# intel/edge-video-analytics-microservice

Measured on AMD Instinct MI355X. Metric: pre-processed frames/sec (1080p NV12→512² NCHW fp32) 1–8 GPU; % HBM peak, higher is better.
Workload: dtype u8->f32; 1 GPU; C2: 32x 1920x1080 NV12 (pitch 1920, device-resident) -> 32x3x512x512 fp32 NCHW, range [0,1] + mean/std; items_per_launch=32, src=1920x1080 NV12, dst=512x512, pool_sets=5, pool_bytes=1000980480, launches_in_flight=3, parallelism=streams s mod 1, one process per GPU, no hot-loop collective

## Files before the change

### edge-video-analytics-microservice_amd/csrc/evam_pp.hip

```cpp
#include <hip/hip_runtime.h>

#include <algorithm>
#include <cmath>
#include <cstdarg>
#include <cstddef>
#include <cstdint>
#include <cstdio>
#include <cstring>
#include <map>
#include <tuple>
#include <mutex>
#include <string>
#include <type_traits>
#include <vector>
#include <immintrin.h>

#include "../../include/evam_pp.h"

#define EVAM_HD __host__ __device__
#include "evam_geom.h"
#include "evam_rings.h"
#include "evam_clip_simd.h"
#include "evam_jpeg_dec.h"
#include "evam_track.h"
// ... 1323 lines not shown
        }
        asm volatile("" ::: "memory");
        int v[3][PX];
        if (cur.pad || (kAblate & 2)) {
#pragma unroll
            for (int j = 0; j < PX; j++) { v[0][j] = fb0; v[1][j] = fo1; v[2][j] = fb2; }
        } else {
            uint32_t NA[PX][3], NB[PX][3];
            const bool shareC = kYUV && cur.stA && cur.stB && !cur.stCB;
            if (shareC) {
                if constexpr (kYUV) hrow2(buf, buf + oY1, buf + oC0, buf + oV0, NA, NB);
            } else {
                if (cur.stA) hrow(buf, buf + oC0, buf + oV0, NA);
                else {
#pragma unroll
                    for (int j = 0; j < PX; j++)
#pragma unroll
                        for (int ch = 0; ch < 3; ch++) NA[j][ch] = cur.ya == pa ? HA[j][ch] : HB[j][ch];
                }
                if (cur.stB) hrow(buf + oY1, buf + (cur.stCB ? oC1 : oC0), buf + (cur.stCB ? oV1 : oV0), NB);
                else {
#pragma unroll
                    for (int j = 0; j < PX; j++)
#pragma unroll
                        for (int ch = 0; ch < 3; ch++)
                            NB[j][ch] = cur.yb == cur.ya ? NA[j][ch] : (cur.yb == pa ? HA[j][ch] : HB[j][ch]);
                }
            }
            const uint32_t wb0 = (uint32_t)cur.b0, wb1 = (uint32_t)cur.b1;
#pragma unroll
            for (int j = 0; j < PX; j++) {
                const bool padc = wa[j] == 0;
#pragma unroll
                for (int ch = 0; ch < 3; ch++) {
                    const int r = vresize(NA[j][ch], NB[j][ch], wb0, wb1);
                    v[ch][j] = padc ? (ch == 0 ? fb0 : (ch == 1 ? fo1 : fb2)) : r;
                }
            }
            if (REUSE) {
#pragma unroll
                for (int j = 0; j < PX; j++)
#pragma unroll
                    for (int ch = 0; ch < 3; ch++) { HA[j][ch] = NA[j][ch]; HB[j][ch] = NB[j][ch]; }
            }
        }
        store_row(Y, v);
        asm volatile("" ::: "memory");
        pa = na;
        pb = nb;
        cur = nxt;
    }
}

#ifdef EVAM_PP_TRACE
constexpr int kTraceWGs = 16384, kTraceSlots = 12;
__device__ unsigned long long g_evam_trace[kTraceWGs * kTraceSlots];
#define EVAM_STAMP(k)                                                                                  \
    do {                                                                                               \
        unsigned long long t_;                                                                         \
        __builtin_amdgcn_sched_barrier(0);                                                             \
        asm volatile("s_memrealtime %0\n\ts_waitcnt lgkmcnt(0)" : "=s"(t_)::"memory");               \
        __builtin_amdgcn_sched_barrier(0);                                                             \
        if (threadIdx.x == 0 && blockIdx.x < kTraceWGs) g_evam_trace[blockIdx.x * kTraceSlots + (k)] = t_; \
    } while (0)
#define EVAM_TRACE_VAL(k, v)                                                                           \
    do {                                                                                               \
        if (threadIdx.x == 0 && blockIdx.x < kTraceWGs) g_evam_trace[blockIdx.x * kTraceSlots + (k)] = (v); \
    } while (0)
#define EVAM_WSTAMP(k)                                                                                 \
    do {                                                                                               \
        unsigned long long t_;                                                                         \
        __builtin_amdgcn_sched_barrier(0);                                                             \
        asm volatile("s_memrealtime %0\n\ts_waitcnt lgkmcnt(0)" : "=s"(t_)::"memory");               \
        __builtin_amdgcn_sched_barrier(0);                                                             \
        const unsigned w_ = ((blockIdx.z * gridDim.y + blockIdx.y) * gridDim.x + blockIdx.x) * (blockDim.x >> 6) + (threadIdx.x >> 6); \
        if ((threadIdx.x & 63) == 0 && w_ < (unsigned)kTraceWGs) g_evam_trace[w_ * kTraceSlots + (k)] = t_; \
    } while (0)
#define EVAM_WTRACE_VAL(k, v)                                                                          \
    do {                                                                                               \
        const unsigned w_ = ((blockIdx.z * gridDim.y + blockIdx.y) * gridDim.x + blockIdx.x) * (blockDim.x >> 6) + (threadIdx.x >> 6); \
        if ((threadIdx.x & 63) == 0 && w_ < (unsigned)kTraceWGs) g_evam_trace[w_ * kTraceSlots + (k)] = (v); \
    } while (0)
#else
#define EVAM_STAMP(k) do { } while (0)
#define EVAM_TRACE_VAL(k, v) do { } while (0)
#define EVAM_WSTAMP(k) do { } while (0)
#define EVAM_WTRACE_VAL(k, v) do { } while (0)
#endif

static_assert(sizeof(evam_roi) == 20, "evam_roi layout");

struct alignas(64) RoiRec {
    const uint8_t* plane[3];
    int32_t pitch[3];
    uint16_t width, height;
    int32_t x, y, w, h;
    int32_t item;
    uint16_t row0, row1;
};
static_assert(sizeof(RoiRec) == 64, "RoiRec layout");
static_assert(offsetof(RoiRec, x) == 40 && offsetof(RoiRec, item) == 56 && offsetof(RoiRec, row0) == 60, "RoiRec lines");
static_assert(offsetof(evam_roi, h) == offsetof(evam_roi, x) + 12, "evam_roi rect");
struct RecFrame { __m128i l[3]; };

constexpr int kMaxStrips = 32;
constexpr int kSfoot = 64;
constexpr int strip_slot(int fmt, int px) { return px == 1 && fmt != kBGRX ? 512 : 1024; }

struct TParams {
    ItemArg items[kArgItems];
    double scale_x, scale_y;
    const float* lut;
    void* dst;
    int slot_offset, slot_stride;
    int DW, DH;
    int cw, ch, rw, rh, ox, oy;
    int nw;
    int TH, tiles_x, tiles_per_item;
    int wave_bytes;
    int color_rgb;
    uint32_t fill;
    int2 sfoot[kSfoot];
    int nstrips, units;
    int segY, segC;
    int nrY;
    int prio;
    int ahead;
};
static_assert(sizeof(TParams) <= 4000, "strip / band kernel arguments must fit the 4 KB kernarg segment");

struct ProgressPrio {
    int next, q2, q3, level;
    __device__ __forceinline__ ProgressPrio(bool on, int n) : next(on ? n / 4 : -1), q2(n / 2), q3((3 * n) / 4), level(3) {
        if (on) __builtin_amdgcn_s_setprio(3);
    }
    __device__ __forceinline__ void step(int i) {
        if (__builtin_expect(i != next, 1)) return;
        if (level == 3) {
            __builtin_amdgcn_s_setprio(2);
            level = 2;
            next = q2;
        } else if (level == 2) {
            __builtin_amdgcn_s_setprio(1);
            level = 1;
            next = q3;
        } else {
            __builtin_amdgcn_s_setprio(0);
            level = 0;
            next = -1;
        }
    }
};

template <int FMT, int OUT, int D, int PX, int PR, bool NHWC = false>
__global__ __launch_bounds__(512) void evam_pp_strip(const TParams P) {
    static_assert(!NHWC || OUT == 1, "the interleaved strip store is fp32 only");
    constexpr int NS = NHWC ? 1 : 3;
    __shared__ __attribute__((aligned(16))) float lut_s[OUT != 0 ? 768 : 4];
    extern __shared__ __attribute__((aligned(16))) uint8_t smem[];
    static_assert(FMT == kNV12 || FMT == kI420 || FMT == kBGRX, "4:2:0 or BGRx sources");
    static_assert(D >= 1 && D <= 4, "ring depth");
    static_assert(PX == 1 || PX == 2, "pixels per lane");
    constexpr int SLOT = strip_slot(FMT, PX);
    constexpr bool PK = FMT == kBGRX;
    constexpr int NPC = FMT == kI420 ? 2 : (PK ? 0 : 1);
    static_assert(PR == 0 || PR == 1, "paired taps");
    constexpr int NMIN = PR ? (PK ? 1 : 2) : 2 + NPC;
    const int lane = threadIdx.x & 63;
    const int wave = __builtin_amdgcn_readfirstlane(threadIdx.x >> 6);
    if (kAblate & 128) return;
    EVAM_WSTAMP(0);
    const uint8_t *p0, *p1, *p2;
    int pitch0, pitch1, pitch2, x0, y0, index, p_nw, p_DH, p_DW, strip, Y0, Y1;
    int g_ox, g_rw, g_oy, g_rh, g_cw, k_ch, k_rgb;
    double k_scale_x, k_scale_y;
    const float* k_lut;
    int2 sf;
    const int item = blockIdx.z, ty = blockIdx.y;
    const ItemArg& it = P.items[item];
    sf = P.sfoot[min((int)blockIdx.x * 8 + wave, kSfoot - 1)];
    const int p_TH = P.TH;
    p_nw = P.nw; p_DH = P.DH; p_DW = P.DW;
    p0 = it.plane[0];
    p1 = it.plane[1];
    p2 = it.plane[2];
    pitch0 = it.pitch[0]; pitch1 = it.pitch[1]; pitch2 = it.pitch[2];
    x0 = it.x0; y0 = it.y0;
    index = it.index;
    asm volatile("" ::"s"(p_nw), "s"(p_TH), "s"(p_DH), "s"(p_DW), "s"(P.ox), "s"(P.rw), "s"(P.oy), "s"(P.rh),
                 "s"(P.wave_bytes), "s"(p0), "s"(p1), "s"(p2), "s"(pitch0), "s"(pitch1), "s"(pitch2), "s"(x0), "s"(y0),
                 "s"(index), "s"(sf.x), "s"(sf.y), "s"(P.dst), "s"(P.slot_offset), "s"(P.slot_stride));
    k_scale_y = P.scale_y;
    k_ch = P.ch; k_rgb = P.color_rgb;
    k_lut = P.lut;
    asm volatile("" : "+s"(k_scale_y), "+s"(k_ch), "+s"(k_lut), "+s"(k_rgb));
    strip = (int)blockIdx.x * p_nw + wave;
    Y0 = ty * p_TH; Y1 = min(Y0 + p_TH, p_DH);
    g_ox = P.ox; g_rw = P.rw; g_oy = P.oy; g_rh = P.rh; g_cw = P.cw;
    k_scale_x = P.scale_x;
    const int X0 = strip * 64 * PX;
    const bool live = X0 < p_DW;
    const bool cols = live && sf.x >= 0;
    int fsY = 0, nY = 0, fsC = 0, nC = 0;
    if (cols) footprint_chunks(FMT, PK ? 4 : 1, x0 + sf.x, x0 + sf.y, fsY, nY, fsC, nC);
    const int vr0 = max(Y0, g_oy), vr1 = min(Y1, g_oy + g_rh);
    const int n = cols && vr1 > vr0 ? vr1 - vr0 : 0;

    int lr0 = 0, lr1 = 0, lb0 = 0, lb1 = 0;
    if (lane < n) {
        int sy, b0, b1;
        linear_coef(vr0 + lane - g_oy, k_scale_y, k_ch, false, sy, b0, b1);
        lr0 = min(max(sy, 0), k_ch - 1);
        lr1 = min(max(sy + 1, 0), k_ch - 1);
        lb0 = b0 << 8;
        lb1 = b1 << 8;
    }
    const __amdgpu_buffer_rsrc_t rsY = __builtin_amdgcn_make_buffer_rsrc((void*)p0, (short)0, 0x7FFFFFFF, 0x00020000);
    const __amdgpu_buffer_rsrc_t rsU = __builtin_amdgcn_make_buffer_rsrc((void*)p1, (short)0, 0x7FFFFFFF, 0x00020000);
    const __amdgpu_buffer_rsrc_t rsV = __builtin_amdgcn_make_buffer_rsrc((void*)(NPC == 2 ? p2 : p1), (short)0, 0x7FFFFFFF, 0x00020000);
    uint8_t* const wbuf = smem + wave * P.wave_bytes;
    constexpr int SY = PR ? 512 : SLOT;
    constexpr int CB = PR ? 1024 : 2 * SLOT;
    constexpr int SC = PR ? (NPC == 2 ? 256 : 512) : SLOT;
    constexpr int SV = PR ? 512 : 2 * SLOT;
    constexpr int GRP = PR ? (PK ? 1024 : 2048) : 2 * SLOT + 2 * NPC * SLOT;
    constexpr int segY = SY;
    const uint8_t* const pcl = NPC == 2 && PR ? (p1 < p2 ? p1 : p2) : p1;
    const uint32_t dU = (uint32_t)(p1 - pcl), dV = (uint32_t)(p2 - pcl);
    const __amdgpu_buffer_rsrc_t rsC2 = __builtin_amdgcn_make_buffer_rsrc((void*)pcl, (short)0, 0x7FFFFFFF, 0x00020000);
    auto issue = [&](int i, int k) {
        if (kAblate & 16) return;
        const int ya = y0 + __builtin_amdgcn_readlane(lr0, i), yb = y0 + __builtin_amdgcn_readlane(lr1, i);
        uint8_t* e = wbuf + k * GRP;
        if constexpr (PR) {
            const int hi = lane >> 5, c = lane & 31;
            if (c < nY)
                __builtin_amdgcn_raw_ptr_buffer_load_lds(rsY, (__attribute__((address_space(3))) void*)e, 16,
                                                         (uint32_t)((hi ? yb : ya) * pitch0 + fsY + c * 16), 0,
                                                         EVAM_PP_LOAD_AUX, 0);
            if constexpr (NPC == 1) {
                const int ca = ya >> 1, cb = yb >> 1;
                if (c < nC && (!hi || ca != cb))
                    __builtin_amdgcn_raw_ptr_buffer_load_lds(rsU, (__attribute__((address_space(3))) void*)(e + CB), 16,
                                                             (uint32_t)((hi ? cb : ca) * pitch1 + fsC + c * 16), 0,
                                                             EVAM_PP_LOAD_AUX, 0);
            } else if constexpr (NPC == 2) {
                const int ca = ya >> 1, cb = yb >> 1, q = lane >> 4, c4 = lane & 15, r = (q & 1) ? cb : ca;
                const uint32_t off = (q & 2) ? dV + (uint32_t)(r * pitch2) : dU + (uint32_t)(r * pitch1);
                if (c4 < nC && (!(q & 1) || ca != cb))
                    __builtin_amdgcn_raw_ptr_buffer_load_lds(rsC2, (__attribute__((address_space(3))) void*)(e + CB), 16,
                                                             off + (uint32_t)(fsC + c4 * 16), 0, EVAM_PP_LOAD_AUX, 0);
            }
            return;
        }
        const uint32_t vo = (uint32_t)lane * 16u;
        if (lane < nY) {
            __builtin_amdgcn_raw_ptr_buffer_load_lds(rsY, (__attribute__((address_space(3))) void*)e, 16, vo,
                                                     ya * pitch0 + fsY, EVAM_PP_LOAD_AUX, 0);
            __builtin_amdgcn_raw_ptr_buffer_load_lds(rsY, (__attribute__((address_space(3))) void*)(e + segY), 16, vo,
                                                     yb * pitch0 + fsY, EVAM_PP_LOAD_AUX, 0);
        }
        if constexpr (NPC == 0) return;
        const int ca = ya >> 1, cb = yb >> 1;
        if (lane < nC) {
            __builtin_amdgcn_raw_ptr_buffer_load_lds(rsU, (__attribute__((address_space(3))) void*)(e + CB), 16, vo,
                                                     ca * pitch1 + fsC, EVAM_PP_LOAD_AUX, 0);
            if constexpr (NPC == 2)
                __builtin_amdgcn_raw_ptr_buffer_load_lds(rsV, (__attribute__((address_space(3))) void*)(e + CB + SV),
                                                         16, vo, ca * pitch2 + fsC, EVAM_PP_LOAD_AUX, 0);
        }
        if (ca != cb && lane < nC) {
            __builtin_amdgcn_raw_ptr_buffer_load_lds(rsU, (__attribute__((address_space(3))) void*)(e + CB + SC), 16,
                                                     vo, cb * pitch1 + fsC, EVAM_PP_LOAD_AUX, 0);
            if constexpr (NPC == 2)
                __builtin_amdgcn_raw_ptr_buffer_load_lds(rsV, (__attribute__((address_space(3))) void*)(e + CB + SV + SC),
                                                         16, vo, cb * pitch2 + fsC, EVAM_PP_LOAD_AUX, 0);
        }
    };

    const int nthr = p_nw * 64;
    const bool lut_early = nthr >= 256;
    if constexpr (OUT != 0) {
        if (lut_early && wave < 3) {
            const __amdgpu_buffer_rsrc_t rsL = __builtin_amdgcn_make_buffer_rsrc((void*)k_lut, (short)0, 3072, 0x00020000);
            __builtin_amdgcn_raw_ptr_buffer_load_lds(rsL, (__attribute__((address_space(3))) void*)(lut_s + wave * 256), 16,
                                                     (uint32_t)lane * 16u, (k_rgb ? 2 - wave : wave) * 1024, 0, 0);
        }
    }
    const int npro = min(n, D);
    for (int i = 0; i < npro; i++) issue(i, i);
    EVAM_WSTAMP(1);
    EVAM_WTRACE_VAL(5, (unsigned long long)blockIdx.z | ((unsigned long long)strip << 16) |
                           ((unsigned long long)blockIdx.y << 32) | ((unsigned long long)n << 48));

    bool xin[PX], padc[PX];
    uint32_t lY[PX], lC0[PX], lC1[PX], wp[PX], vo[PX];
    bool anyp = false;
    const size_t esz = out_esz(OUT);
#pragma unroll
    for (int j = 0; j < PX; j++) {
        const int X = X0 + lane + 64 * j;
        xin[j] = live && X < p_DW;
        vo[j] = (uint32_t)(xin[j] ? X : 0) * (uint32_t)(NHWC ? 3 * esz : esz);
        lY[j] = lC0[j] = lC1[j] = wp[j] = 0;
        padc[j] = true;
        const int dx = X - g_ox;
        if (cols && xin[j] && dx >= 0 && dx < g_rw) {
            int s0, a0, a1;
            linear_coef(dx, k_scale_x, g_cw, true, s0, a0, a1);
            const int ca = x0 + s0;
            lY[j] = (uint32_t)(ca * (PK ? 4 : 1) - fsY);
            if constexpr (FMT == kNV12) {
                lC0[j] = (uint32_t)(2 * (ca >> 1) - fsC);
                lC1[j] = (uint32_t)(2 * ((ca + 1) >> 1) - fsC);
            } else if constexpr (FMT == kI420) {
                lC0[j] = (uint32_t)((ca >> 1) - fsC);
                lC1[j] = (uint32_t)(((ca + 1) >> 1) - fsC);
            }
            wp[j] = PK ? ((uint32_t)a0 << 4) | ((uint32_t)a1 << 20) : (uint32_t)a0 | ((uint32_t)a1 << 16);
            padc[j] = false;
        }
        anyp |= xin[j] && padc[j];
    }
    const bool anypad = cols && __builtin_amdgcn_ballot_w64(anyp) != 0;
    const bool full = X0 + 64 * (PX - 1) < p_DW;

    const size_t plane = (size_t)p_DW * p_DH;
    uint8_t* const d0 = reinterpret_cast<uint8_t*>(P.dst) + (size_t)(P.slot_offset + index * P.slot_stride) * 3 * plane * esz;
    uint8_t* const d1 = d0 + plane * esz;
    uint8_t* const d2 = d1 + plane * esz;
    const __amdgpu_buffer_rsrc_t rsO0 = __builtin_amdgcn_make_buffer_rsrc((void*)(!NHWC && k_rgb ? d2 : d0), (short)0, 0x7FFFFFFF, 0x00020000);
    const __amdgpu_buffer_rsrc_t rsO1 = __builtin_amdgcn_make_buffer_rsrc((void*)d1, (short)0, 0x7FFFFFFF, 0x00020000);
    const __amdgpu_buffer_rsrc_t rsO2 = __builtin_amdgcn_make_buffer_rsrc((void*)(k_rgb ? d0 : d2), (short)0, 0x7FFFFFFF, 0x00020000);
    const uint32_t fq0 = P.fill & 0xFF, fq1 = (P.fill >> 8) & 0xFF, fq2 = (P.fill >> 16) & 0xFF;
    const uint32_t fsh = OUT != 0 ? 2 : 0;
    const uint32_t fill0 = (k_rgb ? fq2 : fq0) << fsh, fill1 = fq1 << fsh, fill2 = (k_rgb ? fq0 : fq2) << fsh;

    if constexpr (OUT != 0) {
        if (lut_early) {
            if (npro == D) asm volatile("s_waitcnt vmcnt(%0)" ::"n"(NMIN * D) : "memory");
            else vmcnt_exact(NMIN * npro);
            lds_barrier();
        } else {
            for (int idx = threadIdx.x; idx < 768; idx += nthr)
                lut_s[idx] = k_lut[k_rgb ? 512 - (idx & ~255) + (idx & 255) : idx];
            __syncthreads();
        }
    }
    EVAM_WSTAMP(2);
    if (!live) return;
    if (kAblate & 64) {
        asm volatile("s_waitcnt vmcnt(0)" ::: "memory");
        asm volatile("" ::"v"(lY[0]), "v"(lC0[0]), "v"(lC1[0]), "v"(wp[0]), "v"(vo[0]), "v"(lb0), "v"(lb1));
        return;
    }
    const uint8_t* lutb = reinterpret_cast<const uint8_t*>(lut_s);
    const uint8_t* aY[PX];
    const uint8_t* aC0[PX];
    const uint8_t* aC1[PX];
#pragma unroll
    for (int j = 0; j < PX; j++) {
        aY[j] = wbuf + lY[j];
        aC0[j] = wbuf + CB + lC0[j];
        aC1[j] = wbuf + CB + lC1[j];
    }
    uint32_t kb = kKBs, kg = kKGs, kr = kKRs;
    int cvg = kCVG, cug = kCUG;
    asm volatile("" : "+v"(kb), "+v"(kg), "+v"(kr), "+s"(cvg), "+s"(cug));
    auto uvt = [&](uint32_t U, uint32_t V) {
        int gu = __mul24((int)U, cug) + (int)kg;
        asm("" : "+v"(gu));
        return UVs{__umul24(U, (uint32_t)kCUB) + kb, (uint32_t)(__mul24((int)V, cvg) + gu), __umul24(V, (uint32_t)kCVR) + kr};
    };
    auto put = [&](int Y, int j, uint32_t v0, uint32_t v1, uint32_t v2) {
        if (!xin[j]) return;
        if (kAblate & 4) {
            asm volatile("" ::"v"(v0), "v"(v1), "v"(v2));
            return;
        }
        if constexpr (NHWC) {
            const int l0 = (int)*reinterpret_cast<const uint32_t*>(lutb + v0);
            const int l1 = (int)*reinterpret_cast<const uint32_t*>(lutb + 1024 + v1);
            const int l2 = (int)*reinterpret_cast<const uint32_t*>(lutb + 2048 + v2);
            const evam_v3i q = {k_rgb ? l2 : l0, l1, k_rgb ? l0 : l2};
            __builtin_amdgcn_raw_buffer_store_b96(q, rsO0, vo[j] + (uint32_t)(Y * p_DW) * 12u, 0, EVAM_PP_STORE_AUX);
            return;
        }
        const int so = (int)((uint32_t)(Y * p_DW) * (uint32_t)esz);
        if constexpr (OUT == 1) {
            __builtin_amdgcn_raw_buffer_store_b32(*reinterpret_cast<const uint32_t*>(lutb + v0), rsO0, vo[j], so, EVAM_PP_STORE_AUX);
            __builtin_amdgcn_raw_buffer_store_b32(*reinterpret_cast<const uint32_t*>(lutb + 1024 + v1), rsO1, vo[j], so, EVAM_PP_STORE_AUX);
            __builtin_amdgcn_raw_buffer_store_b32(*reinterpret_cast<const uint32_t*>(lutb + 2048 + v2), rsO2, vo[j], so, EVAM_PP_STORE_AUX);
        } else if constexpr (OUT == 2) {
            __builtin_amdgcn_raw_buffer_store_b16(*reinterpret_cast<const uint16_t*>(lutb + v0), rsO0, vo[j], so, EVAM_PP_STORE_AUX);
            __builtin_amdgcn_raw_buffer_store_b16(*reinterpret_cast<const uint16_t*>(lutb + 1024 + v1), rsO1, vo[j], so, EVAM_PP_STORE_AUX);
            __builtin_amdgcn_raw_buffer_store_b16(*reinterpret_cast<const uint16_t*>(lutb + 2048 + v2), rsO2, vo[j], so, EVAM_PP_STORE_AUX);
        } else {
            __builtin_amdgcn_raw_buffer_store_b8((uint8_t)v0, rsO0, vo[j], so, EVAM_PP_STORE_AUX);
            __builtin_amdgcn_raw_buffer_store_b8((uint8_t)v1, rsO1, vo[j], so, EVAM_PP_STORE_AUX);
            __builtin_amdgcn_raw_buffer_store_b8((uint8_t)v2, rsO2, vo[j], so, EVAM_PP_STORE_AUX);
        }
    };
    auto put_fill = [&](int Y) {
#pragma unroll
        for (int j = 0; j < PX; j++) put(Y, j, fill0, fill1, fill2);
    };
    const int ra = n ? vr0 : Y1;
    for (int Y = Y0; Y < ra; Y++) put_fill(Y);

    ProgressPrio prio(P.prio != 0, n);
    const int nst = full ? NS * PX : NS;
    auto row = [&](int i, int kk, auto has_pad) {
        constexpr bool PADC = decltype(has_pad)::value;
        constexpr int SD = D - 1;
        if (SD == 0) {
            asm volatile("s_waitcnt vmcnt(0)" ::: "memory");
        } else if (i >= SD && i + D - 1 < n) {
            if (PX == 1 || !full) asm volatile("s_waitcnt vmcnt(%0)" ::"n"((D - 1) * NMIN + SD * NS) : "memory");
            else asm volatile("s_waitcnt vmcnt(%0)" ::"n"((D - 1) * NMIN + SD * NS * PX) : "memory");
        } else {
            vmcnt_exact(NMIN * (min(i + D - 1, n - 1) - i) + nst * min(i, SD));
        }
#ifdef EVAM_PP_TRACE
        if (i == 0) EVAM_WSTAMP(3);
#endif
        prio.step(i);
        const int Y = vr0 + i;
        const uint32_t wb0 = (uint32_t)__builtin_amdgcn_readlane(lb0, i), wb1 = (uint32_t)__builtin_amdgcn_readlane(lb1, i);
        const int ya = __builtin_amdgcn_readlane(lr0, i), yb = __builtin_amdgcn_readlane(lr1, i);
        const bool share = ((y0 + ya) >> 1) == ((y0 + yb) >> 1);
        if (kAblate & 2) {
            put_fill(Y);
        } else if constexpr (PK) {
            const int eo = kk * GRP;
#pragma unroll
            for (int j = 0; j < PX; j++) {
                const uint32_t* ay = reinterpret_cast<const uint32_t*>(aY[j] + eo);
                const uint32_t qa0 = ay[0], qa1 = ay[1], qb0 = ay[SY / 4], qb1 = ay[SY / 4 + 1];
                uint32_t v[3];
#pragma unroll
                for (int c = 0; c < 3; c++) {
                    const uint32_t sel = 0x0C000C00u | ((uint32_t)(4 + c) << 16) | (uint32_t)c;
                    const uint32_t ha = __builtin_amdgcn_udot2(
                        __builtin_bit_cast(evam_u16x2, __builtin_amdgcn_perm(qa1, qa0, sel)),
                        __builtin_bit_cast(evam_u16x2, wp[j]), 0u, false);
                    const uint32_t hb = __builtin_amdgcn_udot2(
                        __builtin_bit_cast(evam_u16x2, __builtin_amdgcn_perm(qb1, qb0, sel)),
                        __builtin_bit_cast(evam_u16x2, wp[j]), 0u, false);
                    v[c] = vfinal<OUT>(ha, hb, wb0, wb1);
                }
                if constexpr (PADC) {
                    v[0] = padc[j] ? fill0 : v[0];
                    v[1] = padc[j] ? fill1 : v[1];
                    v[2] = padc[j] ? fill2 : v[2];
                }
                put(Y, j, v[0], v[1], v[2]);
            }
        } else {
            const int eo = kk * GRP;
            uint32_t rY[PX][4], rC[PX][2][2], rE[PX][2][2];
            auto raw_c = [&](const uint8_t* a, int o, uint32_t (&c)[2]) {
                c[0] = a[o];
                c[1] = FMT == kNV12 ? a[o + 1] : a[o + SV];
            };
#pragma unroll
            for (int j = 0; j < PX; j++) {
                const uint8_t* ay = aY[j] + eo;
                rY[j][0] = ay[0]; rY[j][1] = ay[1]; rY[j][2] = ay[SY]; rY[j][3] = ay[SY + 1];
                raw_c(aC0[j], eo, rC[j][0]);
                raw_c(aC1[j], eo, rC[j][1]);
            }
            if (!share) {
#pragma unroll
                for (int j = 0; j < PX; j++) {
                    raw_c(aC0[j], eo + SC, rE[j][0]);
                    raw_c(aC1[j], eo + SC, rE[j][1]);
                }
            }
#pragma unroll
            for (int j = 0; j < PX; j++) {
                const UVs tA = uvt(rC[j][0][0], rC[j][0][1]), tB = uvt(rC[j][1][0], rC[j][1][1]);
                const uint32_t yA = luma_term(rY[j][0]), yB = luma_term(rY[j][1]);
                const uint32_t yC = luma_term(rY[j][2]), yD = luma_term(rY[j][3]);
                uint32_t h0[3], h1[3];
                h0[0] = hpass_sat(yA, tA.b, yB, tB.b, wp[j]);
                h0[1] = hpass_sat(yA, tA.g, yB, tB.g, wp[j]);
                h0[2] = hpass_sat(yA, tA.r, yB, tB.r, wp[j]);
                if (share) {
                    h1[0] = hpass_sat(yC, tA.b, yD, tB.b, wp[j]);
                    h1[1] = hpass_sat(yC, tA.g, yD, tB.g, wp[j]);
                    h1[2] = hpass_sat(yC, tA.r, yD, tB.r, wp[j]);
                    asm volatile("; strip: shared chroma row" ::"v"(h1[0]), "v"(h1[1]), "v"(h1[2]));
                } else {
                    const UVs tC = uvt(rE[j][0][0], rE[j][0][1]), tE = uvt(rE[j][1][0], rE[j][1][1]);
                    h1[0] = hpass_sat(yC, tC.b, yD, tE.b, wp[j]);
                    h1[1] = hpass_sat(yC, tC.g, yD, tE.g, wp[j]);
                    h1[2] = hpass_sat(yC, tC.r, yD, tE.r, wp[j]);
                    asm volatile("; strip: two chroma rows" ::"v"(h1[0]), "v"(h1[1]), "v"(h1[2]));
                }
                uint32_t v[3];
#pragma unroll
                for (int c = 0; c < 3; c++) v[c] = vfinal<OUT>(h0[c], h1[c], wb0, wb1);
                if constexpr (PADC) {
                    v[0] = padc[j] ? fill0 : v[0];
                    v[1] = padc[j] ? fill1 : v[1];
                    v[2] = padc[j] ? fill2 : v[2];
                }
                put(Y, j, v[0], v[1], v[2]);
            }
        }
        asm volatile("" ::: "memory");
        if (i + D < n) issue(i + D, kk);
        asm volatile("" ::: "memory");
    };
    auto ring = [&](auto has_pad) {
        for (int i0 = 0; i0 < n; i0 += D) {
#pragma unroll
            for (int kk = 0; kk < D; kk++)
                if (i0 + kk < n) row(i0 + kk, kk, has_pad);
        }
    };
    if (anypad) ring(std::true_type{});
    else ring(std::false_type{});
    for (int Y = max(ra, vr1); Y < Y1; Y++) put_fill(Y);
#ifdef EVAM_PP_TRACE
    asm volatile("s_waitcnt vmcnt(0)" ::: "memory");
    EVAM_WSTAMP(4);
    {
        unsigned xcc;
        asm volatile("s_getreg_b32 %0, hwreg(HW_REG_XCC_ID)" : "=s"(xcc));
        EVAM_WTRACE_VAL(6, (unsigned long long)xcc);
    }
#endif
}

__device__ __forceinline__ void vmcnt_le(int n) {
    n = __builtin_amdgcn_readfirstlane(n);
    asm volatile(
        "s_cmp_lt_i32 %0, 8\n\t"
        "s_cbranch_scc1 5f\n\t"
        "s_cmp_lt_i32 %0, 16\n\t"
        "s_cbranch_scc1 2f\n\t"
        "s_cmp_lt_i32 %0, 32\n\t"
        "s_cbranch_scc1 1f\n\t"
        "s_waitcnt vmcnt(32)\n\t"
        "s_branch 9f\n"
        "1:\n\t"
        "s_waitcnt vmcnt(16)\n\t"
        "s_branch 9f\n"
        "2:\n\t"
        "s_cmp_lt_i32 %0, 12\n\t"
        "s_cbranch_scc1 3f\n\t"
        "s_waitcnt vmcnt(12)\n\t"
        "s_branch 9f\n"
        "3:\n\t"
        "s_waitcnt vmcnt(8)\n\t"
        "s_branch 9f\n"
        "5:\n\t"
        "s_cmp_lt_i32 %0, 4\n\t"
        "s_cbranch_scc1 7f\n\t"
        "s_cmp_lt_i32 %0, 6\n\t"
        "s_cbranch_scc1 6f\n\t"
        "s_waitcnt vmcnt(6)\n\t"
        "s_branch 9f\n"
        "6:\n\t"
        "s_waitcnt vmcnt(4)\n\t"
        "s_branch 9f\n"
        "7:\n\t"
        "s_cmp_lt_i32 %0, 2\n\t"
        "s_cbranch_scc1 8f\n\t"
        "s_cmp_lt_i32 %0, 3\n\t"
        "s_cbranch_scc1 4f\n\t"
        "s_waitcnt vmcnt(3)\n\t"
        "s_branch 9f\n"
        "4:\n\t"
        "s_waitcnt vmcnt(2)\n\t"
        "s_branch 9f\n"
        "8:\n\t"
        "s_cmp_lt_i32 %0, 1\n\t"
        "s_cbranch_scc1 10f\n\t"
        "s_waitcnt vmcnt(1)\n\t"
        "s_branch 9f\n"
        "10:\n\t"
        "s_waitcnt vmcnt(0)\n"
        "9:"
        ::"s"(n)
        : "scc", "memory");
}

template <int FMT, int OUT, int PX, int DD, bool NHWC = false>
__global__ __launch_bounds__(256) void evam_pp_band(const TParams P) {
    static_assert(!NHWC || (OUT == 0 && PX == 4), "the interleaved band store is u8 at four pixels per lane");
    constexpr int NS = NHWC ? 1 : 3;
    __shared__ __attribute__((aligned(16))) float lut_s[OUT == 1 ? 768 : 4];
    extern __shared__ __attribute__((aligned(16))) uint8_t smem[];
    if (kAblate & 128) return;
    static_assert(FMT == kNV12 || FMT == kI420, "4:2:0 sources");
    static_assert(PX == 1 || PX == 2 || PX == 4, "pixels per lane");
    static_assert(!DD || PX == 4, "six-column lanes hold 4 pixels");
    constexpr int NPC = FMT == kI420 ? 2 : 1;
    const int lane = threadIdx.x & 63;
    const int wave = __builtin_amdgcn_readfirstlane(threadIdx.x >> 6);
    EVAM_WSTAMP(0);
    const int item = blockIdx.z, band = blockIdx.y;
    const ItemArg& it = P.items[item];
    const int2 sf = P.sfoot[min((int)blockIdx.x * 8 + wave, kSfoot - 1)];
    const int p_nw = P.nw, p_TH = P.TH, p_DH = P.DH, p_DW = P.DW;
    int p_ns = P.nstrips, k_wb = P.wave_bytes;
    const uint8_t* p0 = it.plane[0];
    const uint8_t* p1 = it.plane[1];
    const uint8_t* p2 = it.plane[2];
    const int pitch0 = it.pitch[0], pitch1 = it.pitch[1], pitch2 = it.pitch[2];
    const int x0 = it.x0, y0 = it.y0;
    double k_scale_y = P.scale_y;
    int k_ch = P.ch, k_rgb = P.color_rgb;
    const float* k_lut = P.lut;
    asm volatile("" : "+s"(k_scale_y), "+s"(k_ch), "+s"(k_lut), "+s"(k_rgb), "+s"(p_ns), "+s"(k_wb)
                 : "s"(p_nw), "s"(p_TH), "s"(p_DH), "s"(p_DW), "s"(P.ox), "s"(P.rw), "s"(P.oy), "s"(P.rh),
                   "s"(P.segY), "s"(P.segC), "s"(P.nrY), "s"(p0), "s"(p1), "s"(p2), "s"(pitch0),
                   "s"(pitch1), "s"(pitch2), "s"(x0), "s"(y0), "s"(it.index), "s"(sf.x), "s"(sf.y));
    const int strip = (int)blockIdx.x * p_nw + wave;
    const bool live = strip < p_ns;
    const int Y0 = band * p_TH, Y1 = min(Y0 + p_TH, p_DH);
    const int X0 = strip * 64 * PX;
    const bool cols = live && sf.x >= 0;
    int fsY = 0, nY = 0, fsC = 0, nC = 0;
    if (cols) footprint_chunks(FMT, 1, x0 + sf.x, x0 + sf.y, fsY, nY, fsC, nC);
    const int vr0 = max(Y0, P.oy), vr1 = min(Y1, P.oy + P.rh);
    const int n = cols && vr1 > vr0 ? vr1 - vr0 : 0;

    int lr0 = 0, lr1 = 0, lb0 = 0, lb1 = 0;
    if (lane < n) {
        int sy, b0, b1;
        linear_coef(vr0 + lane - P.oy, k_scale_y, k_ch, false, sy, b0, b1);
        lr0 = min(max(sy, 0), k_ch - 1);
        lr1 = min(max(sy + 1, 0), k_ch - 1);
        lb0 = b0 << 8;
        lb1 = b1 << 8;
    }
    const __amdgpu_buffer_rsrc_t rsY = __builtin_amdgcn_make_buffer_rsrc((void*)p0, (short)0, 0x7FFFFFFF, 0x00020000);
    const __amdgpu_buffer_rsrc_t rsU = __builtin_amdgcn_make_buffer_rsrc((void*)p1, (short)0, 0x7FFFFFFF, 0x00020000);
    const __amdgpu_buffer_rsrc_t rsV = __builtin_amdgcn_make_buffer_rsrc((void*)(NPC == 2 ? p2 : p1), (short)0, 0x7FFFFFFF, 0x00020000);
    uint8_t* const wbuf = smem + wave * k_wb;
    const int segY = P.segY, segC = P.segC;
    uint8_t* const cbuf = wbuf + P.nrY * segY;
    const int rlo = n ? __builtin_amdgcn_readlane(lr0, 0) : 0;
    const int rhi = n ? __builtin_amdgcn_readlane(lr1, n - 1) : -1;
    const int clo = (y0 + rlo) >> 1;
    int pos = 0, dpos = 0;
    if constexpr (OUT == 1) {
        for (int c0 = wave * 64; c0 < 192; c0 += (int)(blockDim.x >> 6) * 64, pos++) {
            const int c = c0 + lane, sec = c >> 6;
            const int src = ((k_rgb ? 2 - sec : sec) * 64 + (c & 63)) * 16;
            const __amdgpu_buffer_rsrc_t rsL = __builtin_amdgcn_make_buffer_rsrc((void*)k_lut, (short)0, 3072, 0x00020000);
            __builtin_amdgcn_raw_ptr_buffer_load_lds(rsL, (__attribute__((address_space(3))) void*)((uint8_t*)lut_s + c0 * 16),
                                                     16, (uint32_t)src, 0, 0, 0);
        }
    }
    const int lut_pos = pos;
    int rnext = rlo, cprev = -1;
    const int ahead = P.ahead;
    auto issue_to = [&](int rmax) {
        const uint32_t vo = (uint32_t)lane * 16u;
        for (; rnext <= rmax; rnext++) {
            const int r = rnext, ya = y0 + r, c = ya >> 1;
            if (lane < nY)
                __builtin_amdgcn_raw_ptr_buffer_load_lds(rsY, (__attribute__((address_space(3))) void*)(wbuf + (r - rlo) * segY),
                                                         16, vo, ya * pitch0 + fsY, EVAM_PP_LOAD_AUX, 0);
            pos++;
            if (c != cprev) {
                uint8_t* cb = cbuf + (c - clo) * segC;
                if (lane < nC) {
// ... 2649 lines not shown
```

Measured before the change: 992,000 frames/s.

## Streamline strip kernel row loop with steady-state path and batched LUT stores

```diff
diff --git a/edge-video-analytics-microservice_amd/csrc/evam_pp.hip b/edge-video-analytics-microservice_amd/csrc/evam_pp.hip
--- a/edge-video-analytics-microservice_amd/csrc/evam_pp.hip
+++ b/edge-video-analytics-microservice_amd/csrc/evam_pp.hip
@@ -1499,6 +1499,10 @@
     }
 };
 
+#ifndef EVAM_STRIP_OPT
+#define EVAM_STRIP_OPT 15
+#endif
+constexpr int kStripOpt = EVAM_STRIP_OPT;
 template <int FMT, int OUT, int D, int PX, int PR, bool NHWC = false>
 __global__ __launch_bounds__(512) void evam_pp_strip(const TParams P) {
     static_assert(!NHWC || OUT == 1, "the interleaved strip store is fp32 only");
@@ -1561,6 +1565,7 @@
         lr1 = min(max(sy + 1, 0), k_ch - 1);
         lb0 = b0 << 8;
         lb1 = b1 << 8;
+        if (!PK && ((y0 + lr0) >> 1) != ((y0 + lr1) >> 1)) lb0 |= (int)0x80000000u;
     }
     const __amdgpu_buffer_rsrc_t rsY = __builtin_amdgcn_make_buffer_rsrc((void*)p0, (short)0, 0x7FFFFFFF, 0x00020000);
     const __amdgpu_buffer_rsrc_t rsU = __builtin_amdgcn_make_buffer_rsrc((void*)p1, (short)0, 0x7FFFFFFF, 0x00020000);
@@ -1575,22 +1580,26 @@
     const uint8_t* const pcl = NPC == 2 && PR ? (p1 < p2 ? p1 : p2) : p1;
     const uint32_t dU = (uint32_t)(p1 - pcl), dV = (uint32_t)(p2 - pcl);
     const __amdgpu_buffer_rsrc_t rsC2 = __builtin_amdgcn_make_buffer_rsrc((void*)pcl, (short)0, 0x7FFFFFFF, 0x00020000);
+    uint32_t hiM = (lane >> 5) ? ~0u : 0u;
+    asm volatile("" : "+v"(hiM));
+    const uint32_t offL = (uint32_t)((lane & 31) * 16);
+    const bool inY = (lane & 31) < nY;
+    const uint64_t mC = __builtin_amdgcn_ballot_w64((lane & 31) < nC), mClo = __builtin_amdgcn_ballot_w64(lane < min(nC, 32));
     auto issue = [&](int i, int k) {
         if (kAblate & 16) return;
         const int ya = y0 + __builtin_amdgcn_readlane(lr0, i), yb = y0 + __builtin_amdgcn_readlane(lr1, i);
         uint8_t* e = wbuf + k * GRP;
         if constexpr (PR) {
-            const int hi = lane >> 5, c = lane & 31;
-            if (c < nY)
+            if (inY)
                 __builtin_amdgcn_raw_ptr_buffer_load_lds(rsY, (__attribute__((address_space(3))) void*)e, 16,
-                                                         (uint32_t)((hi ? yb : ya) * pitch0 + fsY + c * 16), 0,
-                                                         EVAM_PP_LOAD_AUX, 0);
+                                                         offL + (hiM & (uint32_t)((yb - ya) * pitch0)),
+                                                         ya * pitch0 + fsY, EVAM_PP_LOAD_AUX, 0);
             if constexpr (NPC == 1) {
                 const int ca = ya >> 1, cb = yb >> 1;
-                if (c < nC && (!hi || ca != cb))
+                if (__builtin_amdgcn_inverse_ballot_w64(ca != cb ? mC : mClo))
                     __builtin_amdgcn_raw_ptr_buffer_load_lds(rsU, (__attribute__((address_space(3))) void*)(e + CB), 16,
-                                                             (uint32_t)((hi ? cb : ca) * pitch1 + fsC + c * 16), 0,
-                                                             EVAM_PP_LOAD_AUX, 0);
+                                                             offL + (hiM & (uint32_t)((cb - ca) * pitch1)),
+                                                             ca * pitch1 + fsC, EVAM_PP_LOAD_AUX, 0);
             } else if constexpr (NPC == 2) {
                 const int ca = ya >> 1, cb = yb >> 1, q = lane >> 4, c4 = lane & 15, r = (q & 1) ? cb : ca;
                 const uint32_t off = (q & 2) ? dV + (uint32_t)(r * pitch2) : dU + (uint32_t)(r * pitch1);
@@ -1671,6 +1680,7 @@
     }
     const bool anypad = cols && __builtin_amdgcn_ballot_w64(anyp) != 0;
     const bool full = X0 + 64 * (PX - 1) < p_DW;
+    const bool allin = (kStripOpt & 1) && X0 + 64 * PX <= p_DW;
 
     const size_t plane = (size_t)p_DW * p_DH;
     uint8_t* const d0 = reinterpret_cast<uint8_t*>(P.dst) + (size_t)(P.slot_offset + index * P.slot_stride) * 3 * plane * esz;
@@ -1719,33 +1729,54 @@
         asm("" : "+v"(gu));
         return UVs{__umul24(U, (uint32_t)kCUB) + kb, (uint32_t)(__mul24((int)V, cvg) + gu), __umul24(V, (uint32_t)kCVR) + kr};
     };
+    auto lut_at = [&](int c, uint32_t v) -> uint32_t {
+        if constexpr (OUT == 1) return *reinterpret_cast<const uint32_t*>(lutb + 1024 * c + v);
+        else if constexpr (OUT == 2) return *reinterpret_cast<const uint16_t*>(lutb + 1024 * c + v);
+        else return v;
+    };
+    auto store3 = [&](int Y, int j, uint32_t l0, uint32_t l1, uint32_t l2) {
+        if (kAblate & 4) {
+            asm volatile("" ::"v"(l0), "v"(l1), "v"(l2));
+            return;
+        }
+        if constexpr (NHWC) {
+            const evam_v3i q = {(int)(k_rgb ? l2 : l0), (int)l1, (int)(k_rgb ? l0 : l2)};
+            __builtin_amdgcn_raw_buffer_store_b96(q, rsO0, vo[j] + (uint32_t)(Y * p_DW) * 12u, 0, EVAM_PP_STORE_AUX);
+            return;
+        }
+        const int so = (int)((uint32_t)(Y * p_DW) * (uint32_t)esz);
+        if constexpr (OUT == 1) {
+            __builtin_amdgcn_raw_buffer_store_b32(l0, rsO0, vo[j], so, EVAM_PP_STORE_AUX);
+            __builtin_amdgcn_raw_buffer_store_b32(l1, rsO1, vo[j], so, EVAM_PP_STORE_AUX);
+            __builtin_amdgcn_raw_buffer_store_b32(l2, rsO2, vo[j], so, EVAM_PP_STORE_AUX);
+        } else if constexpr (OUT == 2) {
+            __builtin_amdgcn_raw_buffer_store_b16((uint16_t)l0, rsO0, vo[j], so, EVAM_PP_STORE_AUX);
+            __builtin_amdgcn_raw_buffer_store_b16((uint16_t)l1, rsO1, vo[j], so, EVAM_PP_STORE_AUX);
+            __builtin_amdgcn_raw_buffer_store_b16((uint16_t)l2, rsO2, vo[j], so, EVAM_PP_STORE_AUX);
+        } else {
+            __builtin_amdgcn_raw_buffer_store_b8((uint8_t)l0, rsO0, vo[j], so, EVAM_PP_STORE_AUX);
+            __builtin_amdgcn_raw_buffer_store_b8((uint8_t)l1, rsO1, vo[j], so, EVAM_PP_STORE_AUX);
+            __builtin_amdgcn_raw_buffer_store_b8((uint8_t)l2, rsO2, vo[j], so, EVAM_PP_STORE_AUX);
+        }
+    };
     auto put = [&](int Y, int j, uint32_t v0, uint32_t v1, uint32_t v2) {
         if (!xin[j]) return;
-        if (kAblate & 4) {
-            asm volatile("" ::"v"(v0), "v"(v1), "v"(v2));
-            return;
-        }
-        if constexpr (NHWC) {
-            const int l0 = (int)*reinterpret_cast<const uint32_t*>(lutb + v0);
-            const int l1 = (int)*reinterpret_cast<const uint32_t*>(lutb + 1024 + v1);
-            const int l2 = (int)*reinterpret_cast<const uint32_t*>(lutb + 2048 + v2);
-            const evam_v3i q = {k_rgb ? l2 : l0, l1, k_rgb ? l0 : l2};
-            __builtin_amdgcn_raw_buffer_store_b96(q, rsO0, vo[j] + (uint32_t)(Y * p_DW) * 12u, 0, EVAM_PP_STORE_AUX);
-            return;
-        }
-        const int so = (int)((uint32_t)(Y * p_DW) * (uint32_t)esz);
-        if constexpr (OUT == 1) {
-            __builtin_amdgcn_raw_buffer_store_b32(*reinterpret_cast<const uint32_t*>(lutb + v0), rsO0, vo[j], so, EVAM_PP_STORE_AUX);
-            __builtin_amdgcn_raw_buffer_store_b32(*reinterpret_cast<const uint32_t*>(lutb + 1024 + v1), rsO1, vo[j], so, EVAM_PP_STORE_AUX);
-            __builtin_amdgcn_raw_buffer_store_b32(*reinterpret_cast<const uint32_t*>(lutb + 2048 + v2), rsO2, vo[j], so, EVAM_PP_STORE_AUX);
-        } else if constexpr (OUT == 2) {
-            __builtin_amdgcn_raw_buffer_store_b16(*reinterpret_cast<const uint16_t*>(lutb + v0), rsO0, vo[j], so, EVAM_PP_STORE_AUX);
-            __builtin_amdgcn_raw_buffer_store_b16(*reinterpret_cast<const uint16_t*>(lutb + 1024 + v1), rsO1, vo[j], so, EVAM_PP_STORE_AUX);
-            __builtin_amdgcn_raw_buffer_store_b16(*reinterpret_cast<const uint16_t*>(lutb + 2048 + v2), rsO2, vo[j], so, EVAM_PP_STORE_AUX);
+        store3(Y, j, lut_at(0, v0), lut_at(1, v1), lut_at(2, v2));
+    };
+    auto put_row = [&](int Y, const uint32_t (&v)[PX][3]) {
+        if (allin) {
+            uint32_t l[PX][3];
+#pragma unroll
+            for (int j = 0; j < PX; j++)
+#pragma unroll
+                for (int c = 0; c < 3; c++) l[j][c] = lut_at(c, v[j][c]);
+#pragma unroll
+            for (int j = 0; j < PX; j++) store3(Y, j, l[j][0], l[j][1], l[j][2]);
+            asm volatile("; strip: whole groups");
         } else {
-            __builtin_amdgcn_raw_buffer_store_b8((uint8_t)v0, rsO0, vo[j], so, EVAM_PP_STORE_AUX);
-            __builtin_amdgcn_raw_buffer_store_b8((uint8_t)v1, rsO1, vo[j], so, EVAM_PP_STORE_AUX);
-            __builtin_amdgcn_raw_buffer_store_b8((uint8_t)v2, rsO2, vo[j], so, EVAM_PP_STORE_AUX);
+#pragma unroll
+            for (int j = 0; j < PX; j++) put(Y, j, v[j][0], v[j][1], v[j][2]);
+            asm volatile("; strip: partial group");
         }
     };
     auto put_fill = [&](int Y) {
@@ -1757,12 +1788,13 @@
 
     ProgressPrio prio(P.prio != 0, n);
     const int nst = full ? NS * PX : NS;
-    auto row = [&](int i, int kk, auto has_pad) {
+    auto row = [&](int i, int kk, auto has_pad, auto steady) {
         constexpr bool PADC = decltype(has_pad)::value;
+        constexpr bool STEADY = decltype(steady)::value;
         constexpr int SD = D - 1;
         if (SD == 0) {
             asm volatile("s_waitcnt vmcnt(0)" ::: "memory");
-        } else if (i >= SD && i + D - 1 < n) {
+        } else if (STEADY || (i >= SD && i + D - 1 < n)) {
             if (PX == 1 || !full) asm volatile("s_waitcnt vmcnt(%0)" ::"n"((D - 1) * NMIN + SD * NS) : "memory");
             else asm volatile("s_waitcnt vmcnt(%0)" ::"n"((D - 1) * NMIN + SD * NS * PX) : "memory");
         } else {
@@ -1773,18 +1805,25 @@
 #endif
         prio.step(i);
         const int Y = vr0 + i;
-        const uint32_t wb0 = (uint32_t)__builtin_amdgcn_readlane(lb0, i), wb1 = (uint32_t)__builtin_amdgcn_readlane(lb1, i);
-        const int ya = __builtin_amdgcn_readlane(lr0, i), yb = __builtin_amdgcn_readlane(lr1, i);
-        const bool share = ((y0 + ya) >> 1) == ((y0 + yb) >> 1);
+        const int wr0 = __builtin_amdgcn_readlane(lb0, i);
+        const uint32_t wb0 = (uint32_t)wr0 & 0xFFFFFFu, wb1 = (uint32_t)__builtin_amdgcn_readlane(lb1, i);
+        const bool share = wr0 >= 0;
+        const int eo = kk * GRP;
+        uint32_t v[PX][3];
+        auto pad_select = [&](int j) {
+            if constexpr (PADC) {
+                v[j][0] = padc[j] ? fill0 : v[j][0];
+                v[j][1] = padc[j] ? fill1 : v[j][1];
+                v[j][2] = padc[j] ? fill2 : v[j][2];
+            }
+        };
         if (kAblate & 2) {
             put_fill(Y);
         } else if constexpr (PK) {
-            const int eo = kk * GRP;
 #pragma unroll
             for (int j = 0; j < PX; j++) {
                 const uint32_t* ay = reinterpret_cast<const uint32_t*>(aY[j] + eo);
                 const uint32_t qa0 = ay[0], qa1 = ay[1], qb0 = ay[SY / 4], qb1 = ay[SY / 4 + 1];
-                uint32_t v[3];
 #pragma unroll
                 for (int c = 0; c < 3; c++) {
                     const uint32_t sel = 0x0C000C00u | ((uint32_t)(4 + c) << 16) | (uint32_t)c;
@@ -1794,41 +1833,44 @@
                     const uint32_t hb = __builtin_amdgcn_udot2(
                         __builtin_bit_cast(evam_u16x2, __builtin_amdgcn_perm(qb1, qb0, sel)),
                         __builtin_bit_cast(evam_u16x2, wp[j]), 0u, false);
-                    v[c] = vfinal<OUT>(ha, hb, wb0, wb1);
+                    v[j][c] = vfinal<OUT>(ha, hb, wb0, wb1);
                 }
-                if constexpr (PADC) {
-                    v[0] = padc[j] ? fill0 : v[0];
-                    v[1] = padc[j] ? fill1 : v[1];
-                    v[2] = padc[j] ? fill2 : v[2];
-                }
-                put(Y, j, v[0], v[1], v[2]);
-            }
+                pad_select(j);
+            }
+            put_row(Y, v);
         } else {
-            const int eo = kk * GRP;
-            uint32_t rY[PX][4], rC[PX][2][2], rE[PX][2][2];
-            auto raw_c = [&](const uint8_t* a, int o, uint32_t (&c)[2]) {
-                c[0] = a[o];
-                c[1] = FMT == kNV12 ? a[o + 1] : a[o + SV];
+            struct RawC { uint32_t u, v; };
+            auto raw_c = [&](const uint8_t* a, int o) {
+                RawC r{a[o], FMT == kNV12 ? a[o + 1] : a[o + SV]};
+                if (kStripOpt & 8) asm("" : "+v"(r.u), "+v"(r.v));
+                return r;
             };
+            auto uvc = [&](const RawC& r) { return uvt(r.u, r.v); };
+            uint32_t rY[PX][4];
+            RawC rC[PX][2], rE[PX][2];
 #pragma unroll
             for (int j = 0; j < PX; j++) {
                 const uint8_t* ay = aY[j] + eo;
                 rY[j][0] = ay[0]; rY[j][1] = ay[1]; rY[j][2] = ay[SY]; rY[j][3] = ay[SY + 1];
-                raw_c(aC0[j], eo, rC[j][0]);
-                raw_c(aC1[j], eo, rC[j][1]);
-            }
-            if (!share) {
+                rC[j][0] = raw_c(aC0[j], eo);
+                rC[j][1] = raw_c(aC1[j], eo);
+                if (kStripOpt & 2) {
+                    rE[j][0] = raw_c(aC0[j], eo + SC);
+                    rE[j][1] = raw_c(aC1[j], eo + SC);
+                }
+            }
+            if (!(kStripOpt & 2) && !share) {
 #pragma unroll
                 for (int j = 0; j < PX; j++) {
-                    raw_c(aC0[j], eo + SC, rE[j][0]);
-                    raw_c(aC1[j], eo + SC, rE[j][1]);
+                    rE[j][0] = raw_c(aC0[j], eo + SC);
+                    rE[j][1] = raw_c(aC1[j], eo + SC);
                 }
             }
 #pragma unroll
             for (int j = 0; j < PX; j++) {
-                const UVs tA = uvt(rC[j][0][0], rC[j][0][1]), tB = uvt(rC[j][1][0], rC[j][1][1]);
                 const uint32_t yA = luma_term(rY[j][0]), yB = luma_term(rY[j][1]);
                 const uint32_t yC = luma_term(rY[j][2]), yD = luma_term(rY[j][3]);
+                const UVs tA = uvc(rC[j][0]), tB = uvc(rC[j][1]);
                 uint32_t h0[3], h1[3];
                 h0[0] = hpass_sat(yA, tA.b, yB, tB.b, wp[j]);
                 h0[1] = hpass_sat(yA, tA.g, yB, tB.g, wp[j]);
@@ -1839,32 +1881,32 @@
                     h1[2] = hpass_sat(yC, tA.r, yD, tB.r, wp[j]);
                     asm volatile("; strip: shared chroma row" ::"v"(h1[0]), "v"(h1[1]), "v"(h1[2]));
                 } else {
-                    const UVs tC = uvt(rE[j][0][0], rE[j][0][1]), tE = uvt(rE[j][1][0], rE[j][1][1]);
+                    const UVs tC = uvc(rE[j][0]), tE = uvc(rE[j][1]);
                     h1[0] = hpass_sat(yC, tC.b, yD, tE.b, wp[j]);
                     h1[1] = hpass_sat(yC, tC.g, yD, tE.g, wp[j]);
                     h1[2] = hpass_sat(yC, tC.r, yD, tE.r, wp[j]);
                     asm volatile("; strip: two chroma rows" ::"v"(h1[0]), "v"(h1[1]), "v"(h1[2]));
                 }
-                uint32_t v[3];
-#pragma unroll
-                for (int c = 0; c < 3; c++) v[c] = vfinal<OUT>(h0[c], h1[c], wb0, wb1);
-                if constexpr (PADC) {
-                    v[0] = padc[j] ? fill0 : v[0];
-                    v[1] = padc[j] ? fill1 : v[1];
-                    v[2] = padc[j] ? fill2 : v[2];
-                }
-                put(Y, j, v[0], v[1], v[2]);
-            }
+#pragma unroll
+                for (int c = 0; c < 3; c++) v[j][c] = vfinal<OUT>(h0[c], h1[c], wb0, wb1);
+                pad_select(j);
+            }
+            put_row(Y, v);
         }
         asm volatile("" ::: "memory");
-        if (i + D < n) issue(i + D, kk);
+        if (STEADY || i + D < n) issue(i + D, kk);
         asm volatile("" ::: "memory");
     };
     auto ring = [&](auto has_pad) {
-        for (int i0 = 0; i0 < n; i0 += D) {
+        int i0 = 0;
+        while (i0 < n) {
 #pragma unroll
             for (int kk = 0; kk < D; kk++)
-                if (i0 + kk < n) row(i0 + kk, kk, has_pad);
+                if (i0 + kk < n) row(i0 + kk, kk, has_pad, std::false_type{});
+            for (i0 += D; (kStripOpt & 4) && i0 + 2 * D - 1 < n; i0 += D) {
+#pragma unroll
+                for (int kk = 0; kk < D; kk++) row(i0 + kk, kk, has_pad, std::true_type{});
+            }
         }
     };
     if (anypad) ring(std::true_type{});
```

Measured after the change: 1.016 million frames/s (median of 5 runs). 1.02x the previous value.
